# FutureSDR/FutureSDR

Measured on AMD Instinct MI355X. Metric: MSample/s through 127-tap C32 FIR→decim4→1k-FFT flowgraph @1/2/4/8 GPU, higher is better.
Workload: dtype f32; 1 GPU; fir127_decim4_fft1024; taps1=127, taps2=127, decim=4, fft_len=1024, parallelism=1 independent channels

## Files before the change

futuresdr_amd/csrc/futuresdr_hip.hip:

```cpp
#include <hip/hip_runtime.h>

#include <atomic>
#include <condition_variable>
#include <cstdio>
#include <cstring>
#include <cstdlib>
#include <deque>
#include <mutex>
#include <vector>
#include <algorithm>
#include <cmath>

#include "../../include/futuresdr_hip.h"


static thread_local char g_err[512];
static thread_local const char* g_err_ptr = "";

static void set_err(const char* msg) {
    snprintf(g_err, sizeof(g_err), "%s", msg);
    g_err_ptr = g_err;
}

extern "C" const char* fsdr_last_error(void) { return g_err_ptr; }
// ... 647 lines not shown
    const float2* __restrict__ twid ,
    float* __restrict__ mag_out ,
    int fft_len ,
    int stagger ) {
    static_assert(MDFIR_TILE == 1024, "tile == 1024 decimated outputs");
    static_assert(KKD % 4 == 0, "KKD must be a multiple of 4");
    if (stagger > 0) {
        int loops = (int)(blockIdx.x & 7u) * stagger;
        for (int i = 0; i < loops; i++) __builtin_amdgcn_s_sleep(7);
    }
    const unsigned elemsP = MDFIR_TILE + KKD + 8;
    const unsigned SPm = (elemsP + 31u) & ~31u;
    const unsigned SUB = SPm / 4;
    extern __shared__ __attribute__((aligned(16))) char smem[];
    float* planes = (float*)smem;
    float* s_rtx = planes + 4u * SPm;

    const int tid = threadIdx.x;
    const int lane = tid & 63;
    const int wave = tid >> 6;
    const int r16 = lane & 15;
    const int k4 = lane >> 4;

    for (int i = tid; i < 4 * (KKD + 16); i += MDFIR_BLOCK) {
        int v = i / (KKD + 16), t = i % (KKD + 16);
        s_rtx[i] = (t >= 15 && t < 15 + KKD) ? rtv[v * KKD + (t - 15)] : 0.f;
    }
    __syncthreads();

    const unsigned span = 3 + 4 * elemsP;
    constexpr int NL2 =
        (2 * (MDFIR_TILE + KKD + 8) + 3 + MDFIR_BLOCK - 1) / MDFIR_BLOCK;
    float2 stgA[NL2], stgB[NL2];
    auto load_half = [&](long long tl, int h, float2 (&stg)[NL2]) {
        const long long ib = tl * MDFIR_TILE * 4;
#pragma unroll
        for (int j = 0; j < NL2; j++) {
            unsigned idx = (unsigned)(tid + j * MDFIR_BLOCK);
            unsigned rel = 3 + 4 * (idx >> 1) + 2 * h + (idx & 1u);
            long long g = ib + rel;
            stg[j] = (rel < span && g < n_in_valid)
                         ? in[g] : make_float2(0.f, 0.f);
        }
    };
    auto write_half = [&](const float2 (&stg)[NL2]) {
#pragma unroll
        for (int j = 0; j < NL2; j++) {
            unsigned idx = (unsigned)(tid + j * MDFIR_BLOCK);
            unsigned i = idx >> 1, vloc = idx & 1u;
            if (i < elemsP) {
                unsigned d = (i & 3u) * SUB + (i >> 2);
                planes[vloc * SPm + d] = stg[j].x;
                planes[(2 + vloc) * SPm + d] = stg[j].y;
            }
        }
    };
    const unsigned abase = (unsigned)wave * 64 + 4u * r16;
    const unsigned asub = (unsigned)k4 * SUB;
    auto mfma_half = [&](int h, v4f& cre, v4f& cim) {
#pragma unroll
        for (int vloc = 0; vloc < 2; vloc++) {
            const float* pre = planes + (unsigned)vloc * SPm + asub;
            const float* pim = planes + (unsigned)(2 + vloc) * SPm + asub;
            const int v = 2 * h + vloc;
            float bfrag[KKD / 4];
#pragma unroll
            for (int s = 0; s < KKD / 4; s++)
                bfrag[s] = s_rtx[v * (KKD + 16) + 15 + 4 * s + k4 - r16];
            __builtin_amdgcn_s_setprio(1);
#pragma unroll
            for (int t = 0; t < (KKD / 4) / 4; t++) {
                float4 ar = *(const float4*)&pre[abase + 4 * t];
                float4 ai = *(const float4*)&pim[abase + 4 * t];
                cre = __builtin_amdgcn_mfma_f32_16x16x4f32(
                    ar.x, bfrag[4 * t], cre, 0, 0, 0);
                cim = __builtin_amdgcn_mfma_f32_16x16x4f32(
                    ai.x, bfrag[4 * t], cim, 0, 0, 0);
                cre = __builtin_amdgcn_mfma_f32_16x16x4f32(
                    ar.y, bfrag[4 * t + 1], cre, 0, 0, 0);
                cim = __builtin_amdgcn_mfma_f32_16x16x4f32(
                    ai.y, bfrag[4 * t + 1], cim, 0, 0, 0);
                cre = __builtin_amdgcn_mfma_f32_16x16x4f32(
                    ar.z, bfrag[4 * t + 2], cre, 0, 0, 0);
                cim = __builtin_amdgcn_mfma_f32_16x16x4f32(
                    ai.z, bfrag[4 * t + 2], cim, 0, 0, 0);
                cre = __builtin_amdgcn_mfma_f32_16x16x4f32(
                    ar.w, bfrag[4 * t + 3], cre, 0, 0, 0);
                cim = __builtin_amdgcn_mfma_f32_16x16x4f32(
                    ai.w, bfrag[4 * t + 3], cim, 0, 0, 0);
            }
#pragma unroll
            for (int s = (KKD / 4) & ~3; s < KKD / 4; s++) {
                float a_re = pre[abase + s];
                float a_im = pim[abase + s];
                cre = __builtin_amdgcn_mfma_f32_16x16x4f32(
                    a_re, bfrag[s], cre, 0, 0, 0);
                cim = __builtin_amdgcn_mfma_f32_16x16x4f32(
                    a_im, bfrag[s], cim, 0, 0, 0);
            }
            __builtin_amdgcn_s_setprio(0);
        }
    };

    load_half(blockIdx.x, 0, stgA);
    for (long long tile = blockIdx.x;
         tile * (long long)MDFIR_TILE < n_out; tile += gridDim.x) {
        const long long out_base = tile * MDFIR_TILE;
        v4f cre = {0.f, 0.f, 0.f, 0.f};
        v4f cim = {0.f, 0.f, 0.f, 0.f};
        write_half(stgA);
        __syncthreads();
        load_half(tile, 1, stgB);
        mfma_half(0, cre, cim);
        __syncthreads();
        write_half(stgB);
        __syncthreads();
        if ((tile + gridDim.x) * (long long)MDFIR_TILE < n_out)
            load_half(tile + gridDim.x, 0, stgA);
        mfma_half(1, cre, cim);
        __syncthreads();
        float2* ping = (float2*)planes;
        float2* pong = ping + 1024;
        const unsigned Lm = (unsigned)fft_len - 1u;
#pragma unroll
        for (int q = 0; q < 4; q++) {
            int row = k4 * 4 + q;
            unsigned pos = wave * 256 + 16 * row + r16;
            ping[(pos & ~Lm) | fft_swz(pos & Lm)] =
                make_float2(cre[q], cim[q]);
        }
        __syncthreads();
        {
            const int F = 1024 / fft_len;
            const int tpf = MDFIR_BLOCK / F;
            const int fl = tid / tpf, tfr = tid - fl * tpf;
            float2* res = fft_pow2_fwd(ping + (size_t)fl * fft_len,
                                       pong + (size_t)fl * fft_len, twid,
                                       fft_len, tfr, tpf) -
                          (size_t)fl * fft_len;
            for (int i = tid; i < 1024; i += MDFIR_BLOCK) {
                long long o = out_base + i;
                if (o < n_out) {
                    float2 v =
                        res[((unsigned)i & ~Lm) | fft_swz((unsigned)i & Lm)];
                    if (out) out[o] = v;
                    if (mag_out) mag_out[o] = v.x * v.x + v.y * v.y;
                }
            }
        }
        __syncthreads();
    }
}

template <int KKD>
__global__ __launch_bounds__(MDFIR_BLOCK) void k_decim4_fft_mfma_ap_tpl(
    const float2* __restrict__ in, float2* __restrict__ out,
    const float* __restrict__ rtv ,
    long long n_out, long long n_in_valid,
    const float2* __restrict__ twid ,
    float* __restrict__ mag_out ,
    int fft_len) {
    static_assert(KKD % 4 == 0, "KKD must be a multiple of 4");
    const unsigned elemsP = MDFIR_TILE + KKD + 8;
    const unsigned SPm = (elemsP + 31u) & ~31u;
    const unsigned SUB = SPm / 4;
    extern __shared__ __attribute__((aligned(16))) char smem[];
    float* planes = (float*)smem;
    float* s_rtx = planes + 8u * SPm;

    const int tid = threadIdx.x;
    const int lane = tid & 63;
    const int wave = tid >> 6;
    const int r16 = lane & 15;
    const int k4 = lane >> 4;

    for (int i = tid; i < 4 * (KKD + 16); i += MDFIR_BLOCK) {
        int v = i / (KKD + 16), t = i % (KKD + 16);
        s_rtx[i] = (t >= 15 && t < 15 + KKD) ? rtv[v * KKD + (t - 15)] : 0.f;
    }
    __syncthreads();

    constexpr unsigned GROUPS = (MDFIR_TILE + KKD + 8) + 1;
    constexpr int NG = (GROUPS + MDFIR_BLOCK - 1) / MDFIR_BLOCK;
    float4 stqa[NG], stqb[NG];
    auto load_all = [&](long long tl) {
        const long long qb = tl * MDFIR_TILE;
#pragma unroll
        for (int j = 0; j < NG; j++) {
            unsigned q = (unsigned)(tid + j * MDFIR_BLOCK);
            float4 a = make_float4(0.f, 0.f, 0.f, 0.f);
            float4 b = make_float4(0.f, 0.f, 0.f, 0.f);
            if (q < GROUPS) {
                long long xq = (qb + q) * 4;
                if (xq + 3 < n_in_valid) {
                    a = *(const float4*)&in[xq];
                    b = *(const float4*)&in[xq + 2];
                } else {
                    float2 e0 = (xq < n_in_valid) ? in[xq]
                                                  : make_float2(0.f, 0.f);
                    float2 e1 = (xq + 1 < n_in_valid)
                                    ? in[xq + 1] : make_float2(0.f, 0.f);
                    float2 e2 = (xq + 2 < n_in_valid)
                                    ? in[xq + 2] : make_float2(0.f, 0.f);
                    float2 e3 = (xq + 3 < n_in_valid)
                                    ? in[xq + 3] : make_float2(0.f, 0.f);
                    a = make_float4(e0.x, e0.y, e1.x, e1.y);
                    b = make_float4(e2.x, e2.y, e3.x, e3.y);
                }
            }
            stqa[j] = a;
            stqb[j] = b;
        }
    };
    auto write_all = [&]() {
#pragma unroll
        for (int j = 0; j < NG; j++) {
            unsigned q = (unsigned)(tid + j * MDFIR_BLOCK);
            if (q >= GROUPS) continue;
            float4 a = stqa[j], b = stqb[j];
            if (q >= 1) {
                unsigned d1 = ((q - 1) & 3u) * SUB + ((q - 1) >> 2);
                planes[1u * SPm + d1] = a.x;
                planes[5u * SPm + d1] = a.y;
                planes[2u * SPm + d1] = a.z;
                planes[6u * SPm + d1] = a.w;
                planes[3u * SPm + d1] = b.x;
                planes[7u * SPm + d1] = b.y;
            }
            if (q < elemsP) {
                unsigned d0 = (q & 3u) * SUB + (q >> 2);
                planes[0u * SPm + d0] = b.z;
                planes[4u * SPm + d0] = b.w;
            }
        }
    };
    const unsigned abase = (unsigned)wave * 64 + 4u * r16;
    const unsigned asub = (unsigned)k4 * SUB;

    load_all(blockIdx.x);
    for (long long tile = blockIdx.x;
         tile * (long long)MDFIR_TILE < n_out; tile += gridDim.x) {
        const long long out_base = tile * MDFIR_TILE;
        v4f cre = {0.f, 0.f, 0.f, 0.f};
        v4f cim = {0.f, 0.f, 0.f, 0.f};
        write_all();
        __syncthreads();
        if ((tile + gridDim.x) * (long long)MDFIR_TILE < n_out)
            load_all(tile + gridDim.x);
#pragma unroll
        for (int v = 0; v < 4; v++) {
            const float* pre = planes + (unsigned)v * SPm + asub;
            const float* pim = planes + (4u + v) * SPm + asub;
            float bfrag[KKD / 4];
#pragma unroll
            for (int s = 0; s < KKD / 4; s++)
                bfrag[s] = s_rtx[v * (KKD + 16) + 15 + 4 * s + k4 - r16];
            __builtin_amdgcn_s_setprio(1);
#pragma unroll
            for (int t = 0; t < (KKD / 4) / 4; t++) {
                float4 ar = *(const float4*)&pre[abase + 4 * t];
                float4 ai = *(const float4*)&pim[abase + 4 * t];
                cre = __builtin_amdgcn_mfma_f32_16x16x4f32(
                    ar.x, bfrag[4 * t], cre, 0, 0, 0);
                cim = __builtin_amdgcn_mfma_f32_16x16x4f32(
                    ai.x, bfrag[4 * t], cim, 0, 0, 0);
                cre = __builtin_amdgcn_mfma_f32_16x16x4f32(
                    ar.y, bfrag[4 * t + 1], cre, 0, 0, 0);
                cim = __builtin_amdgcn_mfma_f32_16x16x4f32(
                    ai.y, bfrag[4 * t + 1], cim, 0, 0, 0);
                cre = __builtin_amdgcn_mfma_f32_16x16x4f32(
                    ar.z, bfrag[4 * t + 2], cre, 0, 0, 0);
                cim = __builtin_amdgcn_mfma_f32_16x16x4f32(
                    ai.z, bfrag[4 * t + 2], cim, 0, 0, 0);
                cre = __builtin_amdgcn_mfma_f32_16x16x4f32(
                    ar.w, bfrag[4 * t + 3], cre, 0, 0, 0);
                cim = __builtin_amdgcn_mfma_f32_16x16x4f32(
                    ai.w, bfrag[4 * t + 3], cim, 0, 0, 0);
            }
#pragma unroll
            for (int s = (KKD / 4) & ~3; s < KKD / 4; s++) {
                float a_re = pre[abase + s];
                float a_im = pim[abase + s];
                cre = __builtin_amdgcn_mfma_f32_16x16x4f32(
                    a_re, bfrag[s], cre, 0, 0, 0);
                cim = __builtin_amdgcn_mfma_f32_16x16x4f32(
                    a_im, bfrag[s], cim, 0, 0, 0);
            }
            __builtin_amdgcn_s_setprio(0);
        }
        __syncthreads();
        float2* ping = (float2*)planes;
        float2* pong = ping + 1024;
        const unsigned Lm = (unsigned)fft_len - 1u;
#pragma unroll
        for (int q = 0; q < 4; q++) {
            int row = k4 * 4 + q;
            unsigned pos = wave * 256 + 16 * row + r16;
            ping[(pos & ~Lm) | fft_swz(pos & Lm)] =
                make_float2(cre[q], cim[q]);
        }
        __syncthreads();
        {
            const int F = 1024 / fft_len;
            const int tpf = MDFIR_BLOCK / F;
            const int fl = tid / tpf, tfr = tid - fl * tpf;
            float2* res = fft_pow2_fwd(ping + (size_t)fl * fft_len,
                                       pong + (size_t)fl * fft_len, twid,
                                       fft_len, tfr, tpf) -
                          (size_t)fl * fft_len;
            for (int i = tid; i < 1024; i += MDFIR_BLOCK) {
                long long o = out_base + i;
                if (o < n_out) {
                    float2 v =
                        res[((unsigned)i & ~Lm) | fft_swz((unsigned)i & Lm)];
                    if (out) out[o] = v;
                    if (mag_out) mag_out[o] = v.x * v.x + v.y * v.y;
                }
            }
        }
        __syncthreads();
    }
}

__device__ __forceinline__ unsigned rev4_10(unsigned i) {
    unsigned r = 0;
#pragma unroll
    for (int d = 0; d < 5; d++) {
        r = (r << 2) | (i & 3u);
        i >>= 2;
    }
    return r;
}

template <int KKD>
__global__ __launch_bounds__(MDFIR_BLOCK) void k_decim4_fft_mfma_ws_tpl(
    const float2* __restrict__ in, float2* __restrict__ out,
    const float* __restrict__ rtv, long long n_out, long long n_in_valid,
    const float2* __restrict__ twid ,
    float* __restrict__ mag_out) {
    static_assert(KKD % 4 == 0, "KKD must be a multiple of 4");
    const unsigned elemsP = MDFIR_TILE + KKD + 8;
    const unsigned SPm = (elemsP + 31u) & ~31u;
    const unsigned SUB = SPm / 4;
    extern __shared__ __attribute__((aligned(16))) char smem[];
    float* planes = (float*)smem;
    float* s_rtx = planes + 8u * SPm;
    float2* fbuf = (float2*)(s_rtx + 4 * (KKD + 16));

    const int tid = threadIdx.x;
    const int lane = tid & 63;
    const int wave = tid >> 6;
    const int r16 = lane & 15;
    const int k4 = lane >> 4;

    for (int i = tid; i < 4 * (KKD + 16); i += MDFIR_BLOCK) {
        int v = i / (KKD + 16), t = i % (KKD + 16);
        s_rtx[i] = (t >= 15 && t < 15 + KKD) ? rtv[v * KKD + (t - 15)] : 0.f;
    }
    __syncthreads();

    constexpr unsigned GROUPS = (MDFIR_TILE + KKD + 8) + 1;
    constexpr int NG = (GROUPS + MDFIR_BLOCK - 1) / MDFIR_BLOCK;
    float4 stqa[NG], stqb[NG];
    auto load_all = [&](long long tl) {
        const long long qb = tl * MDFIR_TILE;
#pragma unroll
        for (int j = 0; j < NG; j++) {
            unsigned q = (unsigned)(tid + j * MDFIR_BLOCK);
            float4 a = make_float4(0.f, 0.f, 0.f, 0.f);
            float4 b = make_float4(0.f, 0.f, 0.f, 0.f);
            if (q < GROUPS) {
                long long xq = (qb + q) * 4;
                if (xq + 3 < n_in_valid) {
                    a = *(const float4*)&in[xq];
                    b = *(const float4*)&in[xq + 2];
                } else {
                    float2 e0 = (xq < n_in_valid) ? in[xq]
                                                  : make_float2(0.f, 0.f);
                    float2 e1 = (xq + 1 < n_in_valid)
                                    ? in[xq + 1] : make_float2(0.f, 0.f);
                    float2 e2 = (xq + 2 < n_in_valid)
                                    ? in[xq + 2] : make_float2(0.f, 0.f);
                    float2 e3 = (xq + 3 < n_in_valid)
                                    ? in[xq + 3] : make_float2(0.f, 0.f);
                    a = make_float4(e0.x, e0.y, e1.x, e1.y);
                    b = make_float4(e2.x, e2.y, e3.x, e3.y);
                }
            }
            stqa[j] = a;
            stqb[j] = b;
        }
    };
    auto write_all = [&]() {
#pragma unroll
        for (int j = 0; j < NG; j++) {
            unsigned q = (unsigned)(tid + j * MDFIR_BLOCK);
            if (q >= GROUPS) continue;
            float4 a = stqa[j], b = stqb[j];
            if (q >= 1) {
                unsigned d1 = ((q - 1) & 3u) * SUB + ((q - 1) >> 2);
                planes[1u * SPm + d1] = a.x;
                planes[5u * SPm + d1] = a.y;
                planes[2u * SPm + d1] = a.z;
                planes[6u * SPm + d1] = a.w;
                planes[3u * SPm + d1] = b.x;
                planes[7u * SPm + d1] = b.y;
            }
            if (q < elemsP) {
                unsigned d0 = (q & 3u) * SUB + (q >> 2);
                planes[0u * SPm + d0] = b.z;
                planes[4u * SPm + d0] = b.w;
            }
        }
    };
    const unsigned abase = (unsigned)wave * 64 + 4u * r16;
    const unsigned asub = (unsigned)k4 * SUB;
    auto mfma_vloc = [&](int v, v4f& cre, v4f& cim, int g0, int g1,
                         bool tail) {
        const float* pre = planes + (unsigned)v * SPm + asub;
        const float* pim = planes + (4u + v) * SPm + asub;
        float bfrag[KKD / 4];
#pragma unroll
        for (int s = 0; s < KKD / 4; s++)
            bfrag[s] = s_rtx[v * (KKD + 16) + 15 + 4 * s + k4 - r16];
        __builtin_amdgcn_s_setprio(1);
#pragma unroll
        for (int t = 0; t < (KKD / 4) / 4; t++) {
            if (t < g0 || t >= g1) continue;
            float4 ar = *(const float4*)&pre[abase + 4 * t];
            float4 ai = *(const float4*)&pim[abase + 4 * t];
            cre = __builtin_amdgcn_mfma_f32_16x16x4f32(ar.x, bfrag[4 * t],
                                                       cre, 0, 0, 0);
            cim = __builtin_amdgcn_mfma_f32_16x16x4f32(ai.x, bfrag[4 * t],
                                                       cim, 0, 0, 0);
            cre = __builtin_amdgcn_mfma_f32_16x16x4f32(
                ar.y, bfrag[4 * t + 1], cre, 0, 0, 0);
            cim = __builtin_amdgcn_mfma_f32_16x16x4f32(
                ai.y, bfrag[4 * t + 1], cim, 0, 0, 0);
            cre = __builtin_amdgcn_mfma_f32_16x16x4f32(
                ar.z, bfrag[4 * t + 2], cre, 0, 0, 0);
            cim = __builtin_amdgcn_mfma_f32_16x16x4f32(
                ai.z, bfrag[4 * t + 2], cim, 0, 0, 0);
            cre = __builtin_amdgcn_mfma_f32_16x16x4f32(
                ar.w, bfrag[4 * t + 3], cre, 0, 0, 0);
            cim = __builtin_amdgcn_mfma_f32_16x16x4f32(
                ai.w, bfrag[4 * t + 3], cim, 0, 0, 0);
        }
        if (tail) {
#pragma unroll
            for (int s = (KKD / 4) & ~3; s < KKD / 4; s++) {
                float a_re = pre[abase + s];
                float a_im = pim[abase + s];
                cre = __builtin_amdgcn_mfma_f32_16x16x4f32(
                    a_re, bfrag[s], cre, 0, 0, 0);
                cim = __builtin_amdgcn_mfma_f32_16x16x4f32(
                    a_im, bfrag[s], cim, 0, 0, 0);
            }
        }
        __builtin_amdgcn_s_setprio(0);
    };
    auto fft_stage = [&](int s) {
        const unsigned L = 1024u >> (2 * s);
        const unsigned m = L >> 2;
        unsigned bf = (unsigned)tid;
        unsigned blk = bf / m, q = bf - blk * m;
        unsigned base = blk * L + q;
        float2 x0 = fbuf[fft_swz(base)];
        float2 x1 = fbuf[fft_swz(base + m)];
        float2 x2 = fbuf[fft_swz(base + 2 * m)];
        float2 x3 = fbuf[fft_swz(base + 3 * m)];
        float2 t0 = f2_add(x0, x2), t1 = f2_sub(x0, x2);
        float2 t2 = f2_add(x1, x3), t3 = f2_sub(x1, x3);
        float2 t3r = make_float2(t3.y, -t3.x);
        float2 w1 = twid[(size_t)q << (2 * s)];
        float2 w2 = cmulf(w1, w1);
        float2 w3 = cmulf(w2, w1);
        fbuf[fft_swz(base)] = f2_add(t0, t2);
        fbuf[fft_swz(base + m)] = cmulf(f2_add(t1, t3r), w1);
        fbuf[fft_swz(base + 2 * m)] = cmulf(f2_sub(t0, t2), w2);
        fbuf[fft_swz(base + 3 * m)] = cmulf(f2_sub(t1, t3r), w3);
    };

    v4f cre = {0.f, 0.f, 0.f, 0.f};
    v4f cim = {0.f, 0.f, 0.f, 0.f};
    bool have_prev = false;
    long long prev_base = 0;
    load_all(blockIdx.x);
    for (long long tile = blockIdx.x;
         tile * (long long)MDFIR_TILE < n_out; tile += gridDim.x) {
        write_all();
        if (have_prev) {
#pragma unroll
            for (int q = 0; q < 4; q++) {
                int row = k4 * 4 + q;
                unsigned pos = wave * 256 + 16 * row + r16;
                fbuf[fft_swz(pos)] = make_float2(cre[q], cim[q]);
            }
        }
        __syncthreads();
        if ((tile + gridDim.x) * (long long)MDFIR_TILE < n_out)
            load_all(tile + gridDim.x);
        cre = (v4f){0.f, 0.f, 0.f, 0.f};
        cim = (v4f){0.f, 0.f, 0.f, 0.f};
        constexpr int G = (KKD / 4) / 4;
        constexpr int GH = G / 2;
        mfma_vloc(0, cre, cim, 0, G, true);
        if (have_prev) fft_stage(0);
        __syncthreads();
        mfma_vloc(1, cre, cim, 0, G, true);
        if (have_prev) fft_stage(1);
        __syncthreads();
        mfma_vloc(2, cre, cim, 0, G, true);
        if (have_prev) fft_stage(2);
        __syncthreads();
        mfma_vloc(3, cre, cim, 0, GH, false);
        if (have_prev) fft_stage(3);
        __syncthreads();
        mfma_vloc(3, cre, cim, GH, G, true);
        if (have_prev) fft_stage(4);
        __syncthreads();
        if (have_prev) {
            for (int i = tid; i < 1024; i += MDFIR_BLOCK) {
                long long o = prev_base + i;
                if (o < n_out) {
                    float2 v = fbuf[fft_swz(rev4_10((unsigned)i))];
                    if (out) out[o] = v;
                    if (mag_out) mag_out[o] = v.x * v.x + v.y * v.y;
                }
            }
        }
        prev_base = tile * MDFIR_TILE;
        have_prev = true;
        __syncthreads();
    }
    if (have_prev) {
#pragma unroll
        for (int q = 0; q < 4; q++) {
            int row = k4 * 4 + q;
            unsigned pos = wave * 256 + 16 * row + r16;
            fbuf[fft_swz(pos)] = make_float2(cre[q], cim[q]);
        }
        __syncthreads();
        for (int s = 0; s < 5; s++) {
            fft_stage(s);
            __syncthreads();
        }
        for (int i = tid; i < 1024; i += MDFIR_BLOCK) {
            long long o = prev_base + i;
            if (o < n_out) {
                float2 v = fbuf[fft_swz(rev4_10((unsigned)i))];
                if (out) out[o] = v;
                if (mag_out) mag_out[o] = v.x * v.x + v.y * v.y;
            }
        }
    }
}

template <int KKD>
__global__ __launch_bounds__(512) void k_decim4_fft_mfma2_tpl(
    const float2* __restrict__ in, float2* __restrict__ out,
    const float* __restrict__ rtv ,
    long long n_out, long long n_in_valid,
    const float2* __restrict__ twid ,
    float* __restrict__ mag_out ) {
    static_assert(true, "two 1024-pt FFT frames per tile");
    static_assert(KKD % 4 == 0, "KKD must be a multiple of 4");
    const unsigned elemsP = 2048 + KKD + 8;
    const unsigned SPm = (elemsP + 31u) & ~31u;
    const unsigned SUB = SPm / 4;
    extern __shared__ __attribute__((aligned(16))) char smem[];
    float* planes = (float*)smem;
    float* s_rtx = planes + 4u * SPm;

    const int tid = threadIdx.x;
    const int lane = tid & 63;
    const int wave = tid >> 6;
    const int r16 = lane & 15;
    const int k4 = lane >> 4;

    for (int i = tid; i < 4 * (KKD + 16); i += 512) {
        int v = i / (KKD + 16), t = i % (KKD + 16);
        s_rtx[i] = (t >= 15 && t < 15 + KKD) ? rtv[v * KKD + (t - 15)] : 0.f;
    }
    __syncthreads();

    const unsigned span = 3 + 4 * elemsP;
    constexpr int NL2 =
        (2 * (2048 + KKD + 8) + 3 + 512 - 1) / 512;
    float2 stgA[NL2], stgB[NL2];
    auto load_half = [&](long long tl, int h, float2 (&stg)[NL2]) {
        const long long ib = tl * 2048 * 4;
#pragma unroll
        for (int j = 0; j < NL2; j++) {
            unsigned idx = (unsigned)(tid + j * 512);
            unsigned rel = 3 + 4 * (idx >> 1) + 2 * h + (idx & 1u);
            long long g = ib + rel;
            stg[j] = (rel < span && g < n_in_valid)
                         ? in[g] : make_float2(0.f, 0.f);
        }
    };
    auto write_half = [&](const float2 (&stg)[NL2]) {
#pragma unroll
        for (int j = 0; j < NL2; j++) {
            unsigned idx = (unsigned)(tid + j * 512);
            unsigned i = idx >> 1, vloc = idx & 1u;
            if (i < elemsP) {
                unsigned d = (i & 3u) * SUB + (i >> 2);
                planes[vloc * SPm + d] = stg[j].x;
                planes[(2 + vloc) * SPm + d] = stg[j].y;
            }
        }
    };
    const unsigned abase = (unsigned)wave * 64 + 4u * r16;
    const unsigned asub = (unsigned)k4 * SUB;
    auto mfma_half = [&](int h, v4f& cre, v4f& cim) {
#pragma unroll
        for (int vloc = 0; vloc < 2; vloc++) {
            const float* pre = planes + (unsigned)vloc * SPm + asub;
            const float* pim = planes + (unsigned)(2 + vloc) * SPm + asub;
            const int v = 2 * h + vloc;
            float bfrag[KKD / 4];
#pragma unroll
            for (int s = 0; s < KKD / 4; s++)
                bfrag[s] = s_rtx[v * (KKD + 16) + 15 + 4 * s + k4 - r16];
            __builtin_amdgcn_s_setprio(1);
#pragma unroll
            for (int t = 0; t < (KKD / 4) / 4; t++) {
                float4 ar = *(const float4*)&pre[abase + 4 * t];
                float4 ai = *(const float4*)&pim[abase + 4 * t];
                cre = __builtin_amdgcn_mfma_f32_16x16x4f32(
                    ar.x, bfrag[4 * t], cre, 0, 0, 0);
                cim = __builtin_amdgcn_mfma_f32_16x16x4f32(
                    ai.x, bfrag[4 * t], cim, 0, 0, 0);
                cre = __builtin_amdgcn_mfma_f32_16x16x4f32(
                    ar.y, bfrag[4 * t + 1], cre, 0, 0, 0);
                cim = __builtin_amdgcn_mfma_f32_16x16x4f32(
                    ai.y, bfrag[4 * t + 1], cim, 0, 0, 0);
                cre = __builtin_amdgcn_mfma_f32_16x16x4f32(
                    ar.z, bfrag[4 * t + 2], cre, 0, 0, 0);
                cim = __builtin_amdgcn_mfma_f32_16x16x4f32(
                    ai.z, bfrag[4 * t + 2], cim, 0, 0, 0);
                cre = __builtin_amdgcn_mfma_f32_16x16x4f32(
                    ar.w, bfrag[4 * t + 3], cre, 0, 0, 0);
                cim = __builtin_amdgcn_mfma_f32_16x16x4f32(
                    ai.w, bfrag[4 * t + 3], cim, 0, 0, 0);
            }
#pragma unroll
            for (int s = (KKD / 4) & ~3; s < KKD / 4; s++) {
                float a_re = pre[abase + s];
                float a_im = pim[abase + s];
                cre = __builtin_amdgcn_mfma_f32_16x16x4f32(
                    a_re, bfrag[s], cre, 0, 0, 0);
                cim = __builtin_amdgcn_mfma_f32_16x16x4f32(
                    a_im, bfrag[s], cim, 0, 0, 0);
            }
            __builtin_amdgcn_s_setprio(0);
        }
    };

    load_half(blockIdx.x, 0, stgA);
    for (long long tile = blockIdx.x;
         tile * (long long)2048 < n_out; tile += gridDim.x) {
        const long long out_base = tile * 2048;
        v4f cre = {0.f, 0.f, 0.f, 0.f};
        v4f cim = {0.f, 0.f, 0.f, 0.f};
        write_half(stgA);
        __syncthreads();
        load_half(tile, 1, stgB);
        mfma_half(0, cre, cim);
        __syncthreads();
        write_half(stgB);
        __syncthreads();
        if ((tile + gridDim.x) * (long long)2048 < n_out)
            load_half(tile + gridDim.x, 0, stgA);
        mfma_half(1, cre, cim);
        __syncthreads();
        float2* fbase = (float2*)planes;
#pragma unroll
        for (int q = 0; q < 4; q++) {
            int row = k4 * 4 + q;
            int pos = wave * 256 + 16 * row + r16;
            int fr = pos >> 10, idx = pos & 1023;
            fbase[fr * 2048 + fft_swz((unsigned)idx)] =
                make_float2(cre[q], cim[q]);
        }
        __syncthreads();
        {
// ... 3262 lines not shown
        if (o + 128 > out_cap) break;
        for (int i = 0; i < 128; i++) {
            float s, c;
            __builtin_sincosf((float)i * freq, &s, &c);
            fsdr_cf32 x = in[T + off + i];
            out[o + i].re = x.re * c - x.im * s;
            out[o + i].im = x.re * s + x.im * c;
        }
        o += 128;
        if (nf < frame_cap) {
            if (frame_off) frame_off[nf] = off;
            if (frame_freq) frame_freq[nf] = freq;
            nf++;
        }
        size_t cur = T + off + 128;
        size_t n_copied = 0;
        while (cur + 80 <= T2 && o + 64 <= out_cap) {
            for (int k = 0; k < 64; k++) {
                float ang =
                    (float)(n_copied * 80 + 128 + 16 + (size_t)k) * freq;
                float s, c;
                __builtin_sincosf(ang, &s, &c);
                fsdr_cf32 x = in[cur + 16 + k];
                out[o + k].re = x.re * c - x.im * s;
                out[o + k].im = x.re * s + x.im * c;
            }
            o += 64;
            cur += 80;
            n_copied++;
        }
    }
    if (num_frames) *num_frames = nf;
    return o;
}


struct fsdr_chain {
    fsdr_filter* fir1 = nullptr;
    fsdr_filter* fir2 = nullptr;
    fsdr_filter* fused = nullptr;
    fsdr_filter* fft = nullptr;
    float2* d_y1 = nullptr;
    float2* d_y2 = nullptr;
    float2* d_null = nullptr;
    size_t y1_cap = 0, y2_cap = 0, null_cap = 0;
};

extern "C" fsdr_chain* fsdr_chain_create(const float* taps1, size_t n_taps1,
                                         const float* taps2, size_t n_taps2,
                                         size_t decim, size_t fft_len) {
    fsdr_chain* c = new fsdr_chain();
    c->fir1 = fsdr_fir_cf32_create(taps1, n_taps1);
    c->fir2 = fsdr_decim_fir_cf32_create(decim, taps2, n_taps2);
    c->fft = fsdr_fft_cf32_create(fft_len, 0, 0, nullptr);
    const char* fz = getenv("FSDR_CHAIN_FUSED");
    if (!fz || atoi(fz) != 0) {
        size_t tg = n_taps1 + n_taps2 - 1;
        std::vector<double> g(tg, 0.0);
        for (size_t a = 0; a < n_taps1; a++)
            for (size_t b = 0; b < n_taps2; b++)
                g[a + b] += (double)taps1[a] * (double)taps2[b];
        std::vector<float> gf(tg);
        for (size_t i = 0; i < tg; i++) gf[i] = (float)g[i];
        c->fused = fsdr_decim_fir_cf32_create(decim, gf.data(), tg);
    }
    if (!c->fir1 || !c->fir2 || !c->fft) {
        fsdr_chain_destroy(c);
        return nullptr;
    }
    return c;
}

extern "C" int fsdr_chain_variant(const fsdr_chain* c, int* fused_kk_mfma) {
    if (!c) { set_err("null chain"); return FSDR_ERR_INVALID; }
    if (fused_kk_mfma) *fused_kk_mfma = c->fused ? c->fused->kk_mfma : 0;
    return FSDR_OK;
}

extern "C" void fsdr_chain_destroy(fsdr_chain* c) {
    if (!c) return;
    fsdr_filter_destroy(c->fir1);
    fsdr_filter_destroy(c->fir2);
    fsdr_filter_destroy(c->fused);
    fsdr_filter_destroy(c->fft);
    if (c->d_y1) (void)hipFree(c->d_y1);
    if (c->d_y2) (void)hipFree(c->d_y2);
    if (c->d_null) (void)hipFree(c->d_null);
    delete c;
}

extern "C" int fsdr_chain_run_dev(fsdr_chain* c, const void* d_in,
                                  size_t n_in, void* d_out, size_t out_cap,
                                  void* d_mag, size_t mag_cap, void* stream,
                                  size_t* consumed, size_t* produced) {
    REQUIRE_GPU();
    if (!c) { set_err("null chain"); return FSDR_ERR_INVALID; }
    hipStream_t st = (hipStream_t)stream;
    const size_t nt1 = c->fir1->n_taps, nt2 = c->fir2->n_taps;
    const size_t D = c->fir2->decim, L = c->fft->fft_len;
    size_t y1 = sat_sub(n_in + 1, nt1);
    size_t y2 = sat_sub(y1 + 1, nt2) / D;
    size_t frames = y2 / L;
    if (d_out && out_cap < frames * L) frames = out_cap / L;
    if (d_mag && mag_cap < frames * L) frames = mag_cap / L;
    size_t prod = frames * L;
    if (consumed) *consumed = prod * D;
    if (produced) *produced = prod;
    if (frames == 0) return FSDR_OK;
    int rc;
    const char* ffz = getenv("FSDR_CHAIN_FFTFUSE");
    const bool fft_fusable =
        (L == 64 || L == 128 || L == 256 || L == 512 || L == 1024);
    if (c->fused && fft_fusable && c->fused->kk_mfma &&
        !c->fft->inverse && !c->fft->fft_shift && c->fft->norm == 0.f &&
        (!ffz || atoi(ffz) != 0)) {
        const int KK = c->fused->kk_mfma;
        long long tiles = ((long long)prod + MDFIR_TILE - 1) / MDFIR_TILE;
        long long cap = grid_cap(8192);
        int grid = (int)std::min<long long>(tiles, cap);
        unsigned elemsP = MDFIR_TILE + KK + 8;
        size_t lds = (4 * (size_t)((elemsP + 31u) & ~31u) +
                      4 * ((size_t)KK + 16)) * sizeof(float);
        float2* spec_dst = (float2*)d_out;
        if (!spec_dst && !d_mag) {
            rc = ensure_dev((void**)&c->d_null, &c->null_cap,
                            (prod + 8) * sizeof(float2));
            if (rc) return rc;
            spec_dst = c->d_null;
        }
        const char* b512 = getenv("FSDR_CHAIN_BLOCK512");
        if (b512 && atoi(b512) != 0 && L == 1024 && KK == 80 &&
            prod % 2048 == 0) {
            long long tiles2 = (long long)prod / 2048;
            int grid2 = (int)std::min<long long>(tiles2, cap);
            unsigned eP2 = 2048 + 80 + 8;
            size_t lds2 = (4 * (size_t)((eP2 + 31u) & ~31u) + 4 * (80 + 16))
                          * sizeof(float);
            hipLaunchKernelGGL(HIP_KERNEL_NAME(k_decim4_fft_mfma2_tpl<80>),
                               dim3(grid2), dim3(512), lds2, st,
                               (const float2*)d_in, spec_dst,
                               c->fused->d_mtaps, (long long)prod,
                               (long long)n_in,
                               (const float2*)c->fft->d_twid,
                               (float*)d_mag);
            HIP_TRY(hipGetLastError());
            return FSDR_OK;
        }
        const char* ws = getenv("FSDR_CHAIN_WS");
        if ((!ws || atoi(ws) != 0) && L == 1024 &&
            ((uintptr_t)d_in & 15u) == 0) {
            unsigned SPm = (elemsP + 31u) & ~31u;
            size_t lds_ws = (8 * (size_t)SPm + 4 * ((size_t)KK + 16)) *
                                sizeof(float) +
                            1024 * sizeof(float2);
#define CHAIN_WS_CASE(KV)                                                 \
    case KV:                                                              \
        hipLaunchKernelGGL(HIP_KERNEL_NAME(k_decim4_fft_mfma_ws_tpl<KV>), \
                           dim3(grid), dim3(MDFIR_BLOCK), lds_ws, st,     \
                           (const float2*)d_in, spec_dst,                 \
                           c->fused->d_mtaps, (long long)prod,            \
                           (long long)n_in,                               \
                           (const float2*)c->fft->d_twid, (float*)d_mag); \
        break;
            switch (KK) {
                CHAIN_WS_CASE(20)
                CHAIN_WS_CASE(32)
                CHAIN_WS_CASE(48)
                CHAIN_WS_CASE(80)
                CHAIN_WS_CASE(144)
                default:
                    set_err("bad chain mfma K");
                    return FSDR_ERR_INVALID;
            }
#undef CHAIN_WS_CASE
            HIP_TRY(hipGetLastError());
            return FSDR_OK;
        }
        const char* ap = getenv("FSDR_CHAIN_ALLPHASE");
        if ((!ap || atoi(ap) != 0) && ((uintptr_t)d_in & 15u) == 0) {
            unsigned SPm = (elemsP + 31u) & ~31u;
            size_t lds_ap =
                (8 * (size_t)SPm + 4 * ((size_t)KK + 16)) * sizeof(float);
#define CHAIN_AP_CASE(KV)                                                 \
    case KV:                                                              \
        hipLaunchKernelGGL(HIP_KERNEL_NAME(k_decim4_fft_mfma_ap_tpl<KV>), \
                           dim3(grid), dim3(MDFIR_BLOCK), lds_ap, st,     \
                           (const float2*)d_in, spec_dst,                 \
                           c->fused->d_mtaps, (long long)prod,            \
                           (long long)n_in,                               \
                           (const float2*)c->fft->d_twid, (float*)d_mag,  \
                           (int)L);                                       \
        break;
            switch (KK) {
                CHAIN_AP_CASE(20)
                CHAIN_AP_CASE(32)
                CHAIN_AP_CASE(48)
                CHAIN_AP_CASE(80)
                CHAIN_AP_CASE(144)
                default:
                    set_err("bad chain mfma K");
                    return FSDR_ERR_INVALID;
            }
#undef CHAIN_AP_CASE
            HIP_TRY(hipGetLastError());
            return FSDR_OK;
        }
        const char* occ8 = getenv("FSDR_CHAIN_OCC8");
        if (occ8 && atoi(occ8) != 0 && KK == 80) {
            hipLaunchKernelGGL(
                HIP_KERNEL_NAME((k_decim4_fft_mfma_tpl<80, 8>)),
                dim3(grid), dim3(MDFIR_BLOCK), lds, st,
                (const float2*)d_in, spec_dst, c->fused->d_mtaps,
                (long long)prod, (long long)n_in,
                (const float2*)c->fft->d_twid, (float*)d_mag, (int)L, 0);
            HIP_TRY(hipGetLastError());
            return FSDR_OK;
        }
        int stagger = 0;
        if (const char* sg = getenv("FSDR_CHAIN_STAGGER"))
            stagger = atoi(sg);
#define CHAIN_TPL_CASE(KV)                                                \
    case KV:                                                              \
        hipLaunchKernelGGL(HIP_KERNEL_NAME(k_decim4_fft_mfma_tpl<KV>),    \
                           dim3(grid), dim3(MDFIR_BLOCK), lds, st,        \
                           (const float2*)d_in, spec_dst,                 \
                           c->fused->d_mtaps, (long long)prod,            \
                           (long long)n_in,                               \
                           (const float2*)c->fft->d_twid, (float*)d_mag,  \
                           (int)L, stagger);                              \
        break;
        switch (KK) {
            CHAIN_TPL_CASE(20)
            CHAIN_TPL_CASE(32)
            CHAIN_TPL_CASE(48)
            CHAIN_TPL_CASE(80)
            CHAIN_TPL_CASE(144)
            default:
                set_err("bad chain mfma K");
                return FSDR_ERR_INVALID;
        }
#undef CHAIN_TPL_CASE
        HIP_TRY(hipGetLastError());
        return FSDR_OK;
    }
    rc = ensure_dev((void**)&c->d_y2, &c->y2_cap,
                    (prod + 8) * sizeof(float2));
    if (rc) return rc;
    float2* out2 = (float2*)d_out;
    if (!out2) {
        rc = ensure_dev((void**)&c->d_null, &c->null_cap,
                        (prod + 8) * sizeof(float2));
        if (rc) return rc;
        out2 = c->d_null;
    }
    if (c->fused) {
        rc = launch_decim_cf32(c->fused, d_in, c->d_y2, prod, n_in, st);
        if (rc) return rc;
    } else {
        size_t y1_need = D - 1 + (prod - 1) * D + nt2;
        rc = ensure_dev((void**)&c->d_y1, &c->y1_cap,
                        (y1_need + 8) * sizeof(float2));
        if (rc) return rc;
        rc = launch_fir_cf32(c->fir1, d_in, c->d_y1, y1_need, n_in, st);
        if (rc) return rc;
        rc = launch_decim_cf32(c->fir2, c->d_y1, c->d_y2, prod, y1_need,
                               st);
        if (rc) return rc;
    }
    rc = launch_fft(c->fft, c->d_y2, out2, frames, st, (float*)d_mag);
    return rc;
}


struct RingBuf {
    void* host = nullptr;
    void* dev = nullptr;
    size_t items = 0;
    hipEvent_t ev = nullptr;
    hipEvent_t free_ev = nullptr;
};

struct fsdr_ring {
    size_t n_buffers, items_per_buffer, item_bytes, reserved;
    std::vector<RingBuf> bufs;
    std::deque<int> empty_q, full_q;
    int writer_cur = -1, reader_cur = -1;
    int prev_buf = -1;
    size_t prev_tail_off = 0;
    size_t carry_items = 0;
    size_t presented_items = 0;
    size_t presented_off = 0;
    std::mutex mu;
    std::condition_variable cv;
    hipStream_t copy_stream = nullptr;
};

extern "C" fsdr_ring* fsdr_ring_create(size_t n_buffers,
                                       size_t items_per_buffer,
                                       size_t item_bytes,
                                       size_t reserved_items) {
    if (!have_gpu()) { set_err("no HIP device"); return nullptr; }
    if (n_buffers < 2 || items_per_buffer == 0 || item_bytes == 0) {
        set_err("invalid ring parameters");
        return nullptr;
    }
    fsdr_ring* r = new fsdr_ring();
    r->n_buffers = n_buffers;
// ... 253 lines not shown
```

Before: 187,700 MSample/s.

## Cache FFT twiddles in LDS, defer output stores, add fast-path tile loads

Adds a shared chain_stage_load helper with a fast unguarded float4 load path for interior tiles, used by both the ap and ws kernels. The ws kernel now stages its per-stage FFT twiddles in LDS instead of reading global memory inside each radix-4 stage. It holds each finished FFT tile's outputs in registers and stores them during the next iteration, overlapping global writes with later compute. It also sets a launch-bounds occupancy hint of 3 blocks. The costs are more LDS per block, extra live registers, and possible spills under the occupancy hint.

```diff
diff --git a/futuresdr_amd/csrc/futuresdr_hip.hip b/futuresdr_amd/csrc/futuresdr_hip.hip
--- a/futuresdr_amd/csrc/futuresdr_hip.hip
+++ b/futuresdr_amd/csrc/futuresdr_hip.hip
@@ -823,6 +823,57 @@
     }
 }
 
+template <int KKD, int NG>
+__device__ __forceinline__ void chain_stage_load(
+    const float2* __restrict__ in, long long tl, long long n_in_valid,
+    int tid, float4 (&stqa)[NG], float4 (&stqb)[NG]) {
+    constexpr unsigned GROUPS = (MDFIR_TILE + KKD + 8) + 1;
+    static_assert(NG == (GROUPS + MDFIR_BLOCK - 1) / MDFIR_BLOCK, "NG");
+    const long long qb = tl * MDFIR_TILE;
+    if ((qb + GROUPS) * 4 <= n_in_valid) {
+        const float4* p = (const float4*)(in + (qb + tid) * 4);
+#pragma unroll
+        for (int j = 0; j < NG; j++) {
+            float4 a = make_float4(0.f, 0.f, 0.f, 0.f);
+            float4 b = make_float4(0.f, 0.f, 0.f, 0.f);
+            if ((unsigned)(j + 1) * MDFIR_BLOCK <= GROUPS ||
+                (unsigned)(tid + j * MDFIR_BLOCK) < GROUPS) {
+                a = p[2 * j * MDFIR_BLOCK];
+                b = p[2 * j * MDFIR_BLOCK + 1];
+            }
+            stqa[j] = a;
+            stqb[j] = b;
+        }
+        return;
+    }
+#pragma unroll
+    for (int j = 0; j < NG; j++) {
+        unsigned q = (unsigned)(tid + j * MDFIR_BLOCK);
+        float4 a = make_float4(0.f, 0.f, 0.f, 0.f);
+        float4 b = make_float4(0.f, 0.f, 0.f, 0.f);
+        if (q < GROUPS) {
+            long long xq = (qb + q) * 4;
+            if (xq + 3 < n_in_valid) {
+                a = *(const float4*)&in[xq];
+                b = *(const float4*)&in[xq + 2];
+            } else {
+                float2 e0 = (xq < n_in_valid) ? in[xq]
+                                              : make_float2(0.f, 0.f);
+                float2 e1 = (xq + 1 < n_in_valid)
+                                ? in[xq + 1] : make_float2(0.f, 0.f);
+                float2 e2 = (xq + 2 < n_in_valid)
+                                ? in[xq + 2] : make_float2(0.f, 0.f);
+                float2 e3 = (xq + 3 < n_in_valid)
+                                ? in[xq + 3] : make_float2(0.f, 0.f);
+                a = make_float4(e0.x, e0.y, e1.x, e1.y);
+                b = make_float4(e2.x, e2.y, e3.x, e3.y);
+            }
+        }
+        stqa[j] = a;
+        stqb[j] = b;
+    }
+}
+
 template <int KKD>
 __global__ __launch_bounds__(MDFIR_BLOCK) void k_decim4_fft_mfma_ap_tpl(
     const float2* __restrict__ in, float2* __restrict__ out,
@@ -855,33 +906,7 @@
     constexpr int NG = (GROUPS + MDFIR_BLOCK - 1) / MDFIR_BLOCK;
     float4 stqa[NG], stqb[NG];
     auto load_all = [&](long long tl) {
-        const long long qb = tl * MDFIR_TILE;
-#pragma unroll
-        for (int j = 0; j < NG; j++) {
-            unsigned q = (unsigned)(tid + j * MDFIR_BLOCK);
-            float4 a = make_float4(0.f, 0.f, 0.f, 0.f);
-            float4 b = make_float4(0.f, 0.f, 0.f, 0.f);
-            if (q < GROUPS) {
-                long long xq = (qb + q) * 4;
-                if (xq + 3 < n_in_valid) {
-                    a = *(const float4*)&in[xq];
-                    b = *(const float4*)&in[xq + 2];
-                } else {
-                    float2 e0 = (xq < n_in_valid) ? in[xq]
-                                                  : make_float2(0.f, 0.f);
-                    float2 e1 = (xq + 1 < n_in_valid)
-                                    ? in[xq + 1] : make_float2(0.f, 0.f);
-                    float2 e2 = (xq + 2 < n_in_valid)
-                                    ? in[xq + 2] : make_float2(0.f, 0.f);
-                    float2 e3 = (xq + 3 < n_in_valid)
-                                    ? in[xq + 3] : make_float2(0.f, 0.f);
-                    a = make_float4(e0.x, e0.y, e1.x, e1.y);
-                    b = make_float4(e2.x, e2.y, e3.x, e3.y);
-                }
-            }
-            stqa[j] = a;
-            stqb[j] = b;
-        }
+        chain_stage_load<KKD, NG>(in, tl, n_in_valid, tid, stqa, stqb);
     };
     auto write_all = [&]() {
 #pragma unroll
@@ -1003,8 +1028,13 @@
     return r;
 }
 
+#define WS_TW_ENTRIES 341
+__host__ __device__ constexpr unsigned ws_tw_off(int s) {
+    return (1024u - (1024u >> (2 * s))) / 3u;
+}
+
 template <int KKD>
-__global__ __launch_bounds__(MDFIR_BLOCK) void k_decim4_fft_mfma_ws_tpl(
+__global__ __launch_bounds__(MDFIR_BLOCK, 3) void k_decim4_fft_mfma_ws_tpl(
     const float2* __restrict__ in, float2* __restrict__ out,
     const float* __restrict__ rtv, long long n_out, long long n_in_valid,
     const float2* __restrict__ twid ,
@@ -1017,6 +1047,7 @@
     float* planes = (float*)smem;
     float* s_rtx = planes + 8u * SPm;
     float2* fbuf = (float2*)(s_rtx + 4 * (KKD + 16));
+    float2* s_tw = fbuf + 1024;
 
     const int tid = threadIdx.x;
     const int lane = tid & 63;
@@ -1028,46 +1059,26 @@
         int v = i / (KKD + 16), t = i % (KKD + 16);
         s_rtx[i] = (t >= 15 && t < 15 + KKD) ? rtv[v * KKD + (t - 15)] : 0.f;
     }
+    for (int i = tid; i < WS_TW_ENTRIES; i += MDFIR_BLOCK) {
+        int s = (i >= 256) + (i >= 320) + (i >= 336) + (i >= 340);
+        s_tw[i] = twid[(size_t)(i - ws_tw_off(s)) << (2 * s)];
+    }
     __syncthreads();
 
     constexpr unsigned GROUPS = (MDFIR_TILE + KKD + 8) + 1;
     constexpr int NG = (GROUPS + MDFIR_BLOCK - 1) / MDFIR_BLOCK;
     float4 stqa[NG], stqb[NG];
     auto load_all = [&](long long tl) {
-        const long long qb = tl * MDFIR_TILE;
+        chain_stage_load<KKD, NG>(in, tl, n_in_valid, tid, stqa, stqb);
+    };
+    auto write_all = [&]() {
 #pragma unroll
         for (int j = 0; j < NG; j++) {
             unsigned q = (unsigned)(tid + j * MDFIR_BLOCK);
-            float4 a = make_float4(0.f, 0.f, 0.f, 0.f);
-            float4 b = make_float4(0.f, 0.f, 0.f, 0.f);
-            if (q < GROUPS) {
-                long long xq = (qb + q) * 4;
-                if (xq + 3 < n_in_valid) {
-                    a = *(const float4*)&in[xq];
-                    b = *(const float4*)&in[xq + 2];
-                } else {
-                    float2 e0 = (xq < n_in_valid) ? in[xq]
-                                                  : make_float2(0.f, 0.f);
-                    float2 e1 = (xq + 1 < n_in_valid)
-                                    ? in[xq + 1] : make_float2(0.f, 0.f);
-                    float2 e2 = (xq + 2 < n_in_valid)
-                                    ? in[xq + 2] : make_float2(0.f, 0.f);
-                    float2 e3 = (xq + 3 < n_in_valid)
-                                    ? in[xq + 3] : make_float2(0.f, 0.f);
-                    a = make_float4(e0.x, e0.y, e1.x, e1.y);
-                    b = make_float4(e2.x, e2.y, e3.x, e3.y);
-                }
-            }
-            stqa[j] = a;
-            stqb[j] = b;
-        }
-    };
-    auto write_all = [&]() {
-#pragma unroll
-        for (int j = 0; j < NG; j++) {
-            unsigned q = (unsigned)(tid + j * MDFIR_BLOCK);
+            float4 a = stqa[j], b = stqb[j];
+            asm volatile("" ::"v"(a.x), "v"(a.y), "v"(a.z), "v"(a.w),
+                         "v"(b.x), "v"(b.y), "v"(b.z), "v"(b.w));
             if (q >= GROUPS) continue;
-            float4 a = stqa[j], b = stqb[j];
             if (q >= 1) {
                 unsigned d1 = ((q - 1) & 3u) * SUB + ((q - 1) >> 2);
                 planes[1u * SPm + d1] = a.x;
@@ -1143,7 +1154,7 @@
         float2 t0 = f2_add(x0, x2), t1 = f2_sub(x0, x2);
         float2 t2 = f2_add(x1, x3), t3 = f2_sub(x1, x3);
         float2 t3r = make_float2(t3.y, -t3.x);
-        float2 w1 = twid[(size_t)q << (2 * s)];
+        float2 w1 = s_tw[ws_tw_off(s) + q];
         float2 w2 = cmulf(w1, w1);
         float2 w3 = cmulf(w2, w1);
         fbuf[fft_swz(base)] = f2_add(t0, t2);
@@ -1156,6 +1167,20 @@
     v4f cim = {0.f, 0.f, 0.f, 0.f};
     bool have_prev = false;
     long long prev_base = 0;
+    float2 held[4] = {};
+    bool have_held = false;
+    long long held_base = 0;
+    auto store_held = [&]() {
+#pragma unroll
+        for (int k = 0; k < 4; k++) {
+            long long o = held_base + tid + k * MDFIR_BLOCK;
+            if (o < n_out) {
+                float2 v = held[k];
+                if (out) out[o] = v;
+                if (mag_out) mag_out[o] = v.x * v.x + v.y * v.y;
+            }
+        }
+    };
     load_all(blockIdx.x);
     for (long long tile = blockIdx.x;
          tile * (long long)MDFIR_TILE < n_out; tile += gridDim.x) {
@@ -1168,6 +1193,7 @@
                 fbuf[fft_swz(pos)] = make_float2(cre[q], cim[q]);
             }
         }
+        if (have_held) store_held();
         __syncthreads();
         if ((tile + gridDim.x) * (long long)MDFIR_TILE < n_out)
             load_all(tile + gridDim.x);
@@ -1191,19 +1217,18 @@
         if (have_prev) fft_stage(4);
         __syncthreads();
         if (have_prev) {
-            for (int i = tid; i < 1024; i += MDFIR_BLOCK) {
-                long long o = prev_base + i;
-                if (o < n_out) {
-                    float2 v = fbuf[fft_swz(rev4_10((unsigned)i))];
-                    if (out) out[o] = v;
-                    if (mag_out) mag_out[o] = v.x * v.x + v.y * v.y;
-                }
-            }
+#pragma unroll
+            for (int k = 0; k < 4; k++)
+                held[k] = fbuf[fft_swz(
+                    rev4_10((unsigned)(tid + k * MDFIR_BLOCK)))];
+            held_base = prev_base;
+            have_held = true;
         }
         prev_base = tile * MDFIR_TILE;
         have_prev = true;
         __syncthreads();
     }
+    if (have_held) store_held();
     if (have_prev) {
 #pragma unroll
         for (int q = 0; q < 4; q++) {
@@ -4772,7 +4797,7 @@
             unsigned SPm = (elemsP + 31u) & ~31u;
             size_t lds_ws = (8 * (size_t)SPm + 4 * ((size_t)KK + 16)) *
                                 sizeof(float) +
-                            1024 * sizeof(float2);
+                            (1024 + WS_TW_ENTRIES) * sizeof(float2);
 #define CHAIN_WS_CASE(KV)                                                 \
     case KV:                                                              \
         hipLaunchKernelGGL(HIP_KERNEL_NAME(k_decim4_fft_mfma_ws_tpl<KV>), \
```

After: 210,500 MSample/s (median of 6 runs). 1.12x the previous value.
